# prototypefund/your-voice-TTS

Hardware: AMD Instinct MI355X
Metric: mel-frames/sec + RTF, Tacotron2 + 60-iter Griffin-Lim, LJSpeech (higher is better)
Workload: dtype f32; 1 GPU; configs[1]: Tacotron2 single sentence, HIP decoder loop + HIP Griffin-Lim 60 iters; sentences_per_gpu=1, L=100, gl_iters=60, model_config=config_tacotron2.json + forward_attn_mask (synthesize.py:86), parallelism=single GPU

## Files before the change

### your-voice-tts_amd/csrc/griffin_lim.hip

```cpp
#include <cmath>
#include <cstdio>
#include <cstdlib>
#include <string>
#include <type_traits>
#include <vector>

#include "gl_fft.h"

#ifndef GLP_SLEEP
#define GLP_SLEEP 1
#endif

using namespace tts;

namespace {

__device__ __forceinline__ double fval(float x) { return (double)x; }
__device__ __forceinline__ double fval(gran_t x) { return (double)__uint_as_float((unsigned)x.v); }
__device__ __forceinline__ void fstore(float* p, double v, unsigned) { *p = (float)v; }
__device__ __forceinline__ void fstore(gran_t* p, double v, unsigned tag) {
    p->v = ((unsigned long long)tag << 32) | (unsigned long long)__float_as_uint((float)v);
}

constexpr int MAG_KT = 64;
// ... 219 lines not shown
    for (int i = ilo; i <= ihi; ++i) {
        const int o = q - i * g.hop;
        y = (float)((double)y + fval(fr[(int64_t)i * g.winp + (o - g.fb)]));
        wss = (float)((double)wss + win2[o]);
    }
    return wss > 1.17549435e-38f ? y / wss : y;
}

constexpr int OLA_MAX = 5;
template <typename FT>
__device__ __forceinline__ float ola_sample_unrolled(const FT* __restrict__ fr, int q, int F, const Geo& g,
                                                     const double* __restrict__ win2) {
    if (q < g.woff) return 0.f;
    int ilo = q - g.woff - g.win + 1;
    ilo = ilo <= 0 ? 0 : (ilo + g.hop - 1) / g.hop;
    int ihi = (q - g.woff) / g.hop;
    if (ihi > F - 1) ihi = F - 1;
    double fv[OLA_MAX], wv[OLA_MAX];
#pragma unroll
    for (int k = 0; k < OLA_MAX; ++k) {
        const int i = ilo + k;
        const int o = q - i * g.hop;
        const bool ok = i <= ihi;
        fv[k] = ok ? fval(fr[(int64_t)i * g.winp + (o - g.fb)]) : 0.0;
        wv[k] = ok ? win2[o] : 0.0;
    }
    float y = 0.f, wss = 0.f;
#pragma unroll
    for (int k = 0; k < OLA_MAX; ++k) {
        y = (float)((double)y + fv[k]);
        wss = (float)((double)wss + wv[k]);
    }
    return wss > 1.17549435e-38f ? y / wss : y;
}

struct MagArgs {
    int mode;
    const float* spec;
    int n_in, Fmax;
    const int* F;
    const double* pinv;
    spec_t* S;
    float min_db, ref_db, power, max_norm;
    int signal_norm, symmetric, clip;
};

__device__ __forceinline__ float denorm_db(float x, const MagArgs& a) {
    float d = x;
    if (a.signal_norm) {
        if (a.symmetric) {
            if (a.clip) d = fminf(fmaxf(d, -a.max_norm), a.max_norm);
            d = ((d + a.max_norm) * -a.min_db / (2.f * a.max_norm)) + a.min_db;
        } else {
            if (a.clip) d = fminf(fmaxf(d, 0.f), a.max_norm);
            d = (d * -a.min_db / a.max_norm) + a.min_db;
        }
    }
    return (d + a.ref_db) * 0.05f;
}
__device__ __forceinline__ float denorm_to_amp(float x, const MagArgs& a) { return powf(10.f, denorm_db(x, a)); }
__device__ __forceinline__ float amp_of_db(float x, const MagArgs& a) { return exp10f(denorm_db(x, a)); }

constexpr int LIN_PER = 16;
__global__ __launch_bounds__(256) void gl_linear_magnitude_kernel(const MagArgs a) {
    const int b = blockIdx.y;
    const int64_t n = (int64_t)a.F[b] * NB;
// ... 598 lines not shown
        }
        if (lane == 0) {
            const int f = base + rank;
            sh[0] = f;
            sh[1] = f - 4 >= base && f + 4 < base + cnt && f >= 5 && f <= Fb - 6;
            if (!__all(ok)) fail(2);
        }
    }
    __syncthreads();
    if (sh[2]) return;
    const int f = sh[0];
    const bool local = sh[1];
    constexpr int PN = NFFT / GL_THREADS;
    const spec_t* Sf = a.S + ((int64_t)b * a.Fmax + f) * NB;
    std::conditional_t<TWO, TwMix, TwRegs> twf;
    twf.load(a.c.tw);
    __shared__ __align__(16) double2 tw_pass[TWO ? TW_LDS : 1];
    if constexpr (TWO) TwMix::fill(tw_pass, a.c.tw);
    double2 tk[4];
    spec_t sk[4];
#pragma unroll
    for (int r = 0; r < 4; ++r) {
        tk[r] = a.c.tw[bin2l(r)];
        sk[r] = Sf[bin2l(r)];
    }
    auto tkf = [&](int r) { return tk[r]; };
    const double2 tnyq = !TWO && tid == 0 ? a.c.tw[NH] : double2{0.0, 0.0};
    const spec_t snyq = tid == 0 ? Sf[NH] : 0.f;
    const int N = g.hop * (Fb - 1);
    extern __shared__ __align__(16) float og[];
    const int og_zero = GL_SLOTS * g.winp;
    __shared__ int rlo[GL_SLOTS], rhi[GL_SLOTS], rpre[GL_SLOTS + 1];
    if (tid < GL_SLOTS) {
        rlo[tid] = 0x7FFFFFFF;
        rhi[tid] = -1;
    }
    if (tid < 2) og[og_zero + tid] = 0.f;
    __syncthreads();
    double wi[PN];
    constexpr int OP = (OLA_MAX + 1) / 2;
    unsigned offp[PN][OP];
    float wssv[PN];
    if (og_zero > 0xFFFF) fail(6);
#pragma unroll
    for (int i = 0; i < PN; ++i) {
        const int n = edge_sample(tid, i);
        const bool sup = n >= g.woff && n < g.woff + g.win;
        wi[i] = sup ? a.c.win[n] : 0.0;
        const int q = reflect_idx(f * g.hop + n - NFFT / 2, N) + NFFT / 2;
        int ilo = q - g.woff - g.win + 1;
        ilo = ilo <= 0 ? 0 : (ilo + g.hop - 1) / g.hop;
        int ihi = (q - g.woff) / g.hop;
        if (ihi > Fb - 1) ihi = Fb - 1;
        const bool any = sup && q >= g.woff;
        float wss = 0.f;
#pragma unroll
        for (int k = 0; k < OP; ++k) offp[i][k] = 0u;
#pragma unroll
        for (int k = 0; k < OLA_MAX; ++k) {
            const int fi = ilo + k;
            const int o = q - fi * g.hop;
            const bool ok = any && fi <= ihi;
            const int sl = fi - f + GL_DMAX, gg = o - g.fb;
            if (ok && (sl < 0 || sl >= GL_SLOTS)) fail(4);
            const bool in = ok && sl >= 0 && sl < GL_SLOTS;
            offp[i][k >> 1] |= (unsigned)(in ? sl * g.winp + gg : og_zero) << (16 * (k & 1));
            if (in) {
                atomicMin(&rlo[sl], gg);
                atomicMax(&rhi[sl], gg);
            }
            wss = (float)((double)wss + (ok ? a.c.win2[o] : 0.0));
        }
        wssv[i] = wss > 1.17549435e-38f ? wss : 1.0f;
    }
    __syncthreads();
    if (tid == 0) {
        int acc = 0;
        for (int sl = 0; sl < GL_SLOTS; ++sl) {
            rpre[sl] = acc;
            acc += rhi[sl] >= 0 ? (rhi[sl] - (rlo[sl] & ~1)) / 2 + 1 : 0;
        }
        rpre[GL_SLOTS] = acc;
        if (acc > GL_PAIRS * GL_THREADS) fail(5);
    }
    __syncthreads();
    unsigned gdst[GL_PAIRS];
#pragma unroll
    for (int m = 0; m < GL_PAIRS; ++m) {
        const int u = tid + m * GL_THREADS;
        gdst[m] = (unsigned)og_zero;
        if (u < rpre[GL_SLOTS]) {
            int sl = 0;
            while (u >= rpre[sl + 1]) ++sl;
            const int g0 = (rlo[sl] & ~1) + 2 * (u - rpre[sl]);
            gdst[m] = (unsigned)(sl * g.winp + g0) | (g0 >= rlo[sl] ? 1u << 30 : 0u) | (g0 + 1 <= rhi[sl] ? 1u << 31 : 0u);
        }
    }
    const int gbase = (f - GL_DMAX) * g.winp * 8;
    auto goff = [&](int m) {
        return (gdst[m] >> 30) ? gbase + (int)(gdst[m] & 0x3FFFFFFFu) * 8 : GL_OOB_OFF;
    };
    auto soff_of = [&](int t, int i) {
        const int e = edge_sample(t, i);
// ... 74 lines not shown
        GL_PHASE(3)
        fft2l_inv(v, buf1, twf);
        GL_PHASE(4)
        if (b == 0 && f == p.drop_f) return;
        const unsigned nt = tag0 | (unsigned)(it + 1);
        const auto rD = buf_rsrc(dst, (unsigned)g.winp * 8);
#pragma unroll
        for (int r = 0; r < PN / 2; ++r) {
            const u32x4 gv = u32x4{__float_as_uint((float)(wi[2 * r] * (v[r].x * (1.0 / NH)))), nt,
                                   __float_as_uint((float)(wi[2 * r + 1] * (v[r].y * (1.0 / NH)))), nt};
            const int e = edge_sample(TWO ? tid_opaque() : tid, 2 * r);
            const int off = e + 1 >= g.woff && e < g.woff + g.win ? (e - g.fb) * 8 : GL_OOB_OFF;
            if (local) __builtin_amdgcn_raw_buffer_store_b128(gv, rD, off, 0, 0);
            else __builtin_amdgcn_raw_buffer_store_b128(gv, rD, off, 0, 0x10);
        }
        GL_PHASE(5)
    }
#undef GL_PHASE
    if (timed)
        for (int k = 0; k < 6; ++k) p.prof[k] = ph[k];
}
__global__ __launch_bounds__(GL_THREADS) void gl_persistent_kernel(const PersArgs p) { gl_persistent_body<false>(p); }
__global__ __launch_bounds__(GL_THREADS) __attribute__((amdgpu_waves_per_eu(2, 2))) void gl_persistent2_kernel(
    const PersArgs p) {
    gl_persistent_body<true>(p);
}

__global__ void gl_gran_to_frames_kernel(const gran_t* in, float* out, int64_t n) {
    const int64_t i = (int64_t)blockIdx.x * blockDim.x + threadIdx.x;
    if (i < n) out[i] = __uint_as_float((unsigned)in[i].v);
}

template <typename FT>
__global__ void gl_ola_kernel(const FinArgs a) {
    const int b = blockIdx.y;
    const int Fb = a.F[b];
    const int N = a.g.hop * (Fb - 1);
    const int p = blockIdx.x * blockDim.x + threadIdx.x;
    if (a.host_status && p == 0 && b == 0) {
        __hip_atomic_store(a.host_status, *a.status, __ATOMIC_RELAXED, __HIP_MEMORY_SCOPE_SYSTEM);
        if (a.host_seq) release_word_system(a.host_seq, a.seq);
    }
    if (p >= N) return;
    const bool bad = a.status && *a.status != 0;
    const FT* fr = static_cast<const FT*>(a.frames) + (int64_t)b * a.Fmax * a.g.winp;
    const Geo& g = a.g;
    const int q = p + NFFT / 2;
    float yv;
    if ((g.win + g.hop - 1) / g.hop <= OLA_MAX && q >= g.woff) {
        const int u = q - g.woff;
        const int ihu = u / g.hop;
        int ilo = u - g.win + 1;
        const bool full = ilo >= 1 && ihu <= Fb - 1;
        ilo = ilo <= 0 ? 0 : (ilo + g.hop - 1) / g.hop;
        const int ihi = ihu > Fb - 1 ? Fb - 1 : ihu;
        double fv[OLA_MAX];
#pragma unroll
        for (int k = 0; k < OLA_MAX; ++k) {
            const int i = ilo + k;
            fv[k] = i <= ihi ? fval(fr[(int64_t)i * g.winp + (q - i * g.hop - g.fb)]) : 0.0;
        }
        float y = 0.f, wss = 0.f;
#pragma unroll
        for (int k = 0; k < OLA_MAX; ++k) y = (float)((double)y + fv[k]);
        if (full) {
            wss = a.wssp[u - ihu * g.hop];
        } else {
            for (int i = ilo; i <= ihi; ++i) wss = (float)((double)wss + a.c.win2[q - i * g.hop]);
        }
        yv = wss > 1.17549435e-38f ? y / wss : y;
    } else {
        yv = ola_sample(fr, q, Fb, g, a.c.win2);
    }
    a.y[(int64_t)b * a.Nmax + p] = bad ? __builtin_nanf("") : yv;
}

constexpr int OLA_R = 4;
__device__ __forceinline__ int div_small(int n, int d, float rd) {
    int qt = (int)((float)n * rd);
    const int r = n - qt * d;
    qt += r >= d ? 1 : 0;
    qt -= r < 0 ? 1 : 0;
    return qt;
}
__global__ __launch_bounds__(256) void gl_ola_multi_kernel(const FinArgs a) {
    const int b = blockIdx.y;
    const int Fb = a.F[b];
    const Geo& g = a.g;
    const int N = g.hop * (Fb - 1);
    const int p0 = blockIdx.x * (256 * OLA_R) + threadIdx.x;
    if (a.host_status && p0 == 0 && b == 0) {
        __hip_atomic_store(a.host_status, *a.status, __ATOMIC_RELAXED, __HIP_MEMORY_SCOPE_SYSTEM);
        if (a.host_seq) release_word_system(a.host_seq, a.seq);
    }
    if (p0 >= N) return;
    const bool bad = a.status && *a.status != 0;
    const float* fr = static_cast<const float*>(a.frames) + (int64_t)b * a.Fmax * g.winp;
    const float rhop = __builtin_amdgcn_rcpf((float)g.hop);
    const int step = g.winp - g.hop;
    float fv[OLA_R][OLA_MAX], wv[OLA_R];
    int ilo[OLA_R], ihi[OLA_R];
#pragma unroll
    for (int j = 0; j < OLA_R; ++j) {
        const int q = p0 + 256 * j + NFFT / 2, u = q - g.woff;
        const int ihu = div_small(u, g.hop, rhop);
        int lo = u - g.win + 1;
        const bool full = lo >= 1 && ihu <= Fb - 1;
        lo = lo <= 0 ? 0 : div_small(lo + g.hop - 1, g.hop, rhop);
        const int hi = p0 + 256 * j < N ? min(ihu, Fb - 1) : -1;
        ilo[j] = lo;
        ihi[j] = hi;
        const int o = lo * step + q - g.fb;
#pragma unroll
        for (int k = 0; k < OLA_MAX; ++k) fv[j][k] = lo + k <= hi ? fr[o + k * step] : 0.f;
        wv[j] = full && hi >= 0 ? a.wssp[u - ihu * g.hop] : -1.f;
    }
#pragma unroll
// ... 29 lines not shown
__device__ __forceinline__ void scan_combine(double& A, double& Bv, double pa, double pb) {
    Bv = fma(pb, A, Bv);
    A = pa * A;
}
__global__ __launch_bounds__(SCAN_THREADS) void preemph_scan_kernel(const float* y, int64_t Nmax, const int* F, int hop,
                                                                    double coef, int apply, int64_t chunk, int64_t look,
                                                                    double* wav) {
    const int b = blockIdx.y;
    const int64_t N = (int64_t)hop * (F[b] - 1);
    const int64_t o0 = (int64_t)blockIdx.x * chunk;
    if (o0 >= N) return;
    const int64_t o1 = o0 + chunk < N ? o0 + chunk : N;
    const float* x = y + (int64_t)b * Nmax;
    double* o = wav + (int64_t)b * Nmax;
    const int tid = threadIdx.x, lane = tid & 63, wave = tid >> 6;
    if (!apply) {
        for (int64_t i = o0 + tid; i < o1; i += SCAN_THREADS) o[i] = (double)x[i];
        return;
    }
    constexpr int TILE = SCAN_THREADS * SCAN_PER, NW = SCAN_THREADS / 64;
    __shared__ double wa[NW], wb[NW];
    double cpow[SCAN_PER + 1];
    cpow[0] = 1.0;
#pragma unroll
    for (int k = 1; k <= SCAN_PER; ++k) cpow[k] = cpow[k - 1] * coef;
    const int64_t s0 = o0 - look > 0 ? ((o0 - look) & ~(int64_t)7) : 0;
    double carry = 0.0;
    for (int64_t t0 = s0; t0 < o1; t0 += TILE) {
        const int64_t base = t0 + (int64_t)tid * SCAN_PER;
        double v = 0.0, loc[SCAN_PER];
#pragma unroll
        for (int k = 0; k < SCAN_PER; ++k) {
            v = (base + k < o1 ? (double)x[base + k] : 0.0) + coef * v;
            loc[k] = v;
        }
        double A = cpow[SCAN_PER], Bv = v;
#pragma unroll
        for (int off = 1; off < 64; off <<= 1) {
            const double pa = __shfl_up(A, off, 64), pb = __shfl_up(Bv, off, 64);
            if (lane >= off) scan_combine(A, Bv, pa, pb);
        }
        if (lane == 63) { wa[wave] = A; wb[wave] = Bv; }
        __syncthreads();
        double WA = lane < NW ? wa[lane] : 1.0, WB = lane < NW ? wb[lane] : 0.0;
#pragma unroll
        for (int off = 1; off < NW; off <<= 1) {
            const double qa = __shfl_up(WA, off, 64), qb = __shfl_up(WB, off, 64);
            if (lane >= off) scan_combine(WA, WB, qa, qb);
        }
        const double win_in = wave == 0 ? carry : __shfl(WA, wave - 1, 64) * carry + __shfl(WB, wave - 1, 64);
        const double tile_end = __shfl(WA, NW - 1, 64) * carry + __shfl(WB, NW - 1, 64);
        const double pa = __shfl_up(A, 1, 64), pb = __shfl_up(Bv, 1, 64);
        const double cin = lane == 0 ? win_in : pa * win_in + pb;
#pragma unroll
        for (int k = 0; k < SCAN_PER; ++k) {
            const int64_t i = base + k;
            if (i >= o0 && i < o1) o[i] = loc[k] + cpow[k + 1] * cin;
        }
        carry = tile_end;
        __syncthreads();
    }
}

void launch_iteration(bool fused, bool wave, const IterArgs& a, hipStream_t s) {
    const dim3 grid(a.Fmax, a.B), block(GL_THREADS);
    if (fused) hipLaunchKernelGGL((gl_iter_kernel<false, true, frame_t>), grid, block, 0, s, a);
// ... 311 lines not shown
            } else {
                FinArgs o = c.fa;
                o.frames = frame_slot(g, c, i);
                launch_ola_frames(o, s);
            }
            launch_iteration(c.fused, g->wave, a, s);
        }
        hipError_t ce = hipGetLastError();
        hipError_t ee = hipStreamEndCapture(s, &graph);
        TTS_HIP(ce);
        TTS_HIP(ee);
        hipGraphExec_t exec = nullptr;
        TTS_HIP(hipGraphInstantiate(&exec, graph, nullptr, nullptr, 0));
        TTS_HIP(hipGraphDestroy(graph));
        it = g->graphs.emplace(key, exec).first;
    }
    TTS_HIP(hipGraphLaunch(it->second, s));
    return TTS_OK;
}

tts_status finish(tts_gl* g, RunCtx& c) {
    hipStream_t s = c.s;
    FinArgs& fa = c.fa;
    if (c.timed) TTS_HIP(hipEventRecord(g->ev_t1, s));
    fa.frames = c.persistent_ran ? static_cast<void*>(g->pgr.p + (size_t)(c.iters & 1) * c.fstride)
                                 : frame_slot(g, c, c.iters);
    fa.status = c.persistent_ran ? g->pstatus : nullptr;
    fa.host_status = c.persistent_ran ? g->host_status : nullptr;
    if (c.persistent_ran && !c.timed) {
        fa.host_seq = g->host_status + 1;
        fa.seq = ++g->seq;
        g->seq_stream = s;
    }
    if (c.persistent_ran)
        hipLaunchKernelGGL(gl_ola_kernel<gran_t>, dim3((c.Nmax + 255) / 256, c.B), dim3(256), 0, s, fa);
    else launch_ola_frames(fa, s);
    fa.status = nullptr;
    fa.host_status = nullptr;
    fa.host_seq = nullptr;
    TTS_HIP(hipGetLastError());
    const double cf = g->cfg.preemphasis, ac = std::fabs(cf);
    int64_t chunk = SCAN_CHUNK, look = 0;
    if (ac > 0.0) {
        const double need = ac < 1.0 ? std::ceil(std::log(1e-22) / std::log(ac)) : 1e30;
        if (need <= (double)(SCAN_THREADS * SCAN_PER - SCAN_CHUNK - 8)) look = (int64_t)need;
        else chunk = c.Nmax;
    }
    const dim3 sgrid((unsigned)((c.Nmax + chunk - 1) / chunk), c.B);
    hipLaunchKernelGGL(preemph_scan_kernel, sgrid, dim3(SCAN_THREADS), 0, s, g->y.p, c.Nmax, c.Fd, g->g.hop, cf,
                       cf != 0.0 ? 1 : 0, chunk, look, c.wav);
    TTS_HIP(hipGetLastError());
    return TTS_OK;
}

tts_status record_last(tts_gl* g, const RunCtx& c) {
    g->last_persistent = c.persistent_ran;
    g->last_path = c.persistent_ran ? TTS_GL_PATH_PERSISTENT : c.fused ? TTS_GL_PATH_FUSED : TTS_GL_PATH_UNFUSED;
    g->last_launches = c.persistent_ran ? 1 : (c.fused ? 1 : 2) * c.iters;
    if (c.timed) {
        TTS_HIP(hipEventRecord(g->ev_done, c.s));
        if (c.s != c.cs) TTS_HIP(hipStreamWaitEvent(c.cs, g->ev_done, 0));
    } else {
        g->last_ms = 0.f;
    }
    g->last_timed = c.timed;
    g->pending = true;
    if (!g->pipeline) TTS_TRY(gl_collect(g));
    g->last_fused = c.fused;
    g->have_last = true;
    g->last_iter = c.ia;
    g->last_fin = c.fa;
    g->last_fstride = c.fstride;
    return TTS_OK;
}

}

namespace tts {

bool gl_persistent_path(tts_gl* g, int B, int Fmax, int frames_total, int iters) {
    if (!(gl_fused_path(g, B, Fmax) && iters > 0 && iters < (1 << 14) && frames_total <= 512 && g->tmo > 0 &&
          !env_is("TTS_RESIDENT", '0')))
        return false;
// ... 106 lines not shown
```

### your-voice-tts_amd/csrc/resident_decoder.hip

```cpp
#include "handoff.h"
#include "resident.h"

namespace tts {
namespace {
using namespace handoff;

__device__ __forceinline__ float lstm_cell16(float pre, float& c) {
    const int k = threadIdx.x;
    const float act = (k >> 2) == 2 ? tanh_cell(pre) : sigmoid_cell(pre);
    const float f = dpp_move<0x104, 0xf>(act, 0.f);
    const float g = dpp_move<0x108, 0xf>(act, 0.f);
    const float o = dpp_move<0x10C, 0xf>(act, 0.f);
    const float c2 = f * c + act * g;
    c = c2;
    return o * tanh_cell(c2);
}
__device__ __forceinline__ float sigmoid_fast(float x) {
    return __builtin_amdgcn_rcpf(1.f + __builtin_amdgcn_exp2f(-x * 1.4426950408889634f));
}

__device__ __forceinline__ float dot4(float4 w, float4 x, float acc) {
    acc = fmaf(w.x, x.x, acc);
    acc = fmaf(w.y, x.y, acc);
    acc = fmaf(w.z, x.z, acc);
    return fmaf(w.w, x.w, acc);
}
__device__ __forceinline__ float4 ld4(const float* p) { return *reinterpret_cast<const float4*>(p); }
__device__ __forceinline__ void pin4(float4& a, float4& b, float4& c, float4& d) {
    asm volatile("" : "+v"(a.x), "+v"(a.y), "+v"(a.z), "+v"(a.w), "+v"(b.x), "+v"(b.y), "+v"(b.z), "+v"(b.w), "+v"(c.x),
                 "+v"(c.y), "+v"(c.z), "+v"(c.w), "+v"(d.x), "+v"(d.y), "+v"(d.z), "+v"(d.w));
}
__device__ __forceinline__ float sum32_dpp(float v) {
    v += dpp_move<0x111, 0xf>(v, 0.f);
    v += dpp_move<0x112, 0xf>(v, 0.f);
    v += dpp_move<0x114, 0xf>(v, 0.f);
    v += dpp_move<0x118, 0xf>(v, 0.f);
    v += dpp_move<0x142, 0xa>(v, 0.f);
    return v;
}

__device__ __forceinline__ int res_window(int k, int nn, int L) {
    if (k == 0) return nn >= 2 ? nn - 2 : nn - 2 + L;
    const int clo = nn >= 1 ? nn - 1 : L - 1, chi = min(nn + 2, L - 1);
    const int p = clo + k - 1;
    return p <= chi ? p : -1;
}
__device__ __forceinline__ int res_candidate(int s, int nn, int np, int L) {
    if (s < 5) return res_window(s, nn, L);
    if (s >= 15) return -1;
    const int p = res_window((s - 5) >> 1, np, L);
    if (p < 0) return -1;
    const int q = p + ((s - 5) & 1);
    return q < L ? q : -1;
}

__device__ __forceinline__ int res_part_slot(int sl, int k) { return sl * 32 + k; }

struct ResWin {
    int cx, clo, chi;
    bool in[4];
    bool iscx[4];
    bool pre, post;
};
// ... 340 lines not shown
            aa[i & 1] = dot4(wa[i], ld4(xh_att + (i - 6) * 128 + ks * 4), aa[i & 1]);                               \
        asm volatile("" ::: "memory");                         \
        _Pragma("unroll") for (int i = 10; i < 14; ++i)                                                             \
            aa[i & 1] = dot4(wa[i], ld4(xh_att + (i - 6) * 128 + ks * 4), aa[i & 1]);                               \
        out = aa[0] + aa[1];                                                                                        \
    }
#define RES_DEC_PARTIAL(out)                                                                                        \
    {                                                                                                               \
        float ad[2] = {0.f, 0.f};                                                                                   \
        _Pragma("unroll 2") for (int i = 8; i < 16; ++i)                                                            \
            ad[i & 1] = dot4(wdl[(i * 16 + r) * 32 + ks], ld4(xh_dec + (i - 8) * 128 + ks * 4), ad[i & 1]);         \
        out = ad[0] + ad[1];                                                                                        \
    }
    float acc_a_next = 0.f;
    if constexpr (!GEN) RES_ATT_PARTIAL(acc_a_next)
    int t = 0;
    for (;; ++t) {
        u64* G = a.gran + (t & 1) * GR_TOTAL;
        u64* const gxs = GEN ? Gx + (t & 1) * GR_TOTAL : G + s_x;
        u64* const gqs = GEN ? Gq + (t & 1) * GR_TOTAL : G + s_q;
        u64* const gcs = GEN ? Gc + (t & 1) * GR_TOTAL : G + s_c;
        u64* const g1s = GEN ? G1 + (t & 1) * GR_TOTAL : G + s_1;
        const unsigned E = (a.salt << 14) | (((unsigned)t & 2047u) << 3);
        const unsigned EP6 = ((a.salt << 14) | (((unsigned)(t - 1) & 2047u) << 3)) + 6u;
        float acc_a, acc_d;
        if constexpr (GEN) {
            RES_ATT_PARTIAL(acc_a)
            RES_DEC_PARTIAL(acc_d)
        } else {
            acc_a = acc_a_next;
        }
        if (tid == 0) { RES_EV(t, 12) }
        if (tid == 192) { RES_EV(t, 13) }
        if (wave < 3) {
            const int gp = s_1 + ((t & 1) ^ 1) * GR_TOTAL;
            bool ok = true;
            if (t == 0) {
                if (wave == 0) {
                    const float4 v = ld4(a.pre1 + lane * 4);
                    xp1[lane * 4] = v.x; xp1[lane * 4 + 1] = v.y; xp1[lane * 4 + 2] = v.z; xp1[lane * 4 + 3] = v.w;
                }
            } else {
                float p0 = 0.f, p1 = 0.f;
                for (int i = 0; i < a.sleep_p1; ++i) __builtin_amdgcn_s_sleep(4);
                if (wave < 2) {
                    ok = sweep_pair(rg, gp + 2 * pk, true, EP6, p0, p1, tmo);
                    xp1[2 * pk] = p0;
                    xp1[2 * pk + 1] = p1;
                } else {
                    ok = sweep_pair(rg, lane == 0 ? gp + PRE : -1, false, EP6, p0, p1, tmo);
                    if (lane == 0 && ok && p0 == 0.f) flags[0] = 1;
                }
            }
            RES_MARK(0);
            if (lane == 0 && !ok) { flags[1] = 1; fail(a.status, 1, t); }
        }
        __syncthreads();
        if (tid == 0) { RES_EV(t, 0) }
        if (flags[0] | flags[1]) break;
        {
            const float4 x = ld4(xp1 + lane * 4);
            u64* gx = gxs;
            if (has_row) {
                const float s0 = wave_sum_dpp(dot4(wp0, x, 0.f));
                if (lane == 0) publish_xcd(gx + r0, E + 1, fmaxf(s0 + bp2, 0.f));
            }
            RES_MARK(1);
            if (wave < 2) {
                for (int i = 0; i < a.sleep_pre2; ++i) __builtin_amdgcn_s_sleep(4);
                float q0, q1;
                const bool ok = sweep_pair(rg, s_x + (t & 1) * GR_TOTAL + 2 * pk, true, E + 1, q0, q1, tmo);
                xpre[2 * pk] = q0;
                xpre[2 * pk + 1] = q1;
                if (!ok && lane == 0) { flags[1] = 1; fail(a.status, 7, t); }
            }
        }
        __syncthreads();
        if (tid == 0) { RES_EV(t, 1) }
        if (flags[1]) break;
        RES_MARK(2);
#pragma unroll
        for (int i = 0; i < 2; ++i) acc_a = dot4(wa[i], ld4(xpre + i * 128 + ks * 4), acc_a);
        acc_a = sum32_dpp(acc_a);
        if (ks == 31) gates[r] = acc_a;
        if constexpr (!GEN) {
            if (t > 0) {
                if (wave >= RES_POLL_WAVES && wave < 2 * RES_POLL_WAVES) xrow[tid - 64 * RES_POLL_WAVES] = op_row;
                if (wave == 2 * RES_POLL_WAVES) xpt[lane] = op_pt;
            }
        }
        __syncthreads();
        RES_MARK(3);
        if (tid < 16) {
            float cs = st[32 + (tid & 3)];
            const float h = lstm_cell16(gates[tid] + st[tid], cs);
            if (tid < 4) {
                st[32 + tid] = cs;
                st[40 + tid] = h;
                publish(G + GR_HATT + 4 * c + tid, E + 2, h);
                if (tid == 0) { RES_EV(t, 2) }
            }
        }
        if constexpr (!GEN) {
            if (t > 0) {
                if (n == n_prev + 1 && n_prev >= 1) {
                    ex = erow[0];
                    erow[0] = erow[1];
                    erow[1] = erow[2];
                    erow[2] = erow[3];
                    if (wave < RES_POLL_WAVES) erow[3] = xrow[tid];
                    else erow[3] = op_own;
                } else if (n != n_prev) {
// ... 393 lines not shown
            if constexpr (!GEN) {
                RES_ATT_PARTIAL(acc_a_next)
                asm volatile("" : "+v"(acc_a_next));
            }
            for (int i = 0; i < a.sleep_hdec; ++i) __builtin_amdgcn_s_sleep(4);
            float h0, h1;
            const bool ok = sweep_pair(rg, (t & 1) * GR_TOTAL + GR_HDEC + 2 * pk, true, E + 5, h0, h1, tmo);
            xh_dec[2 * pk] = h0;
            xh_dec[2 * pk + 1] = h1;
            if (!ok && lane == 0) { flags[1] = 1; fail(a.status, 5, t); }
        }
        __syncthreads();
        if (tid == 0) { RES_EV(t, 6) }
        if (flags[1]) break;
        if constexpr (!GEN) {
            n_prev = n;
            n = flags[6];
        }
        if constexpr (GEN) {
            if (gf & GEN_TA) {
                float sta = gts[0];
#pragma unroll
                for (int k = 1; k < RES_WAVES; ++k) sta += gts[k];
                gu = sigmoidf_(sta + gtb);
            }
        }
        RES_MARK(12);
        long long m0 = 0;
        if (prof && tid == 128) m0 = (long long)wall_clock64();
        {
            const bool stw = stop_cu && wave == 3;
            const float4* wsr = reinterpret_cast<const float4*>(rm) + 6 * 64 + lane;
            float s = 0.f, ss = 0.f;
#pragma unroll
            for (int i = 0; i < 4; ++i) {
                const float4 x = ld4(xh_dec + i * 256 + lane * 4);
                s = dot4(w1[i], x, s);
                if (stw) ss = dot4(wsr[i * 64], x, ss);
            }
#pragma unroll
            for (int i = 4; i < 6; ++i) {
                const float4 x = ld4(xctx + (i - 4) * 256 + lane * 4);
                s = dot4(w1[i], x, s);
                if (stw) ss = dot4(wsr[i * 64], x, ss);
            }
            s = wave_sum_dpp(s);
            u64* g1 = g1s;
            if (has_row && lane == 0) {
                const float p = fmaxf(s + bp1, 0.f);
                publish_xcd(g1 + r0, E + 6, p);
                if (wave == 0) { RES_EV(t, 7) }
                if (xlog) a.pre1[r0] = p;
            }
            if (stw) {
                ss = wave_sum_dpp(ss);
                if (lane == 0) {
                    const float stv = sigmoidf_(ss + st[49]);
                    if (xlog && t < a.hist_cap) a.stop_hist[t] = stv;
                    const float tail = xctx[ENC];
                    int* sst = reinterpret_cast<int*>(st);
                    const int f1 = sst[50] | ((tail > 0.8f && t > L) ? 1 : 0);
                    sst[50] = f1;
                    int nd = 0;
                    if (f1 && t > 2 * L) {
                        sst[51] += 1;
                        if (sst[51] > 20) nd = 1;
                    } else if (t + 1 == a.max_steps) {
                        nd = 1;
                    }
                    if (!nd && t + 1 >= a.hist_cap) {
                        nd = 1;
                        fail(a.status, 100);
                    }
                    if (nd && xlog) {
                        a.done[0] = 1;
                        a.n_steps[0] = t + 1;
                    }
                    publish_xcd(g1 + PRE, E + 6, nd ? 0.f : 1.f);
                }
            }
        }
        if (prof && tid == 128) pacc[13] += (long long)wall_clock64() - m0;
        if constexpr (!GEN) {
            if (wave >= RES_POLL_WAVES) {
                if (n == n_prev + 1 && n_prev >= 1) {
                    const int ro = n + 2 <= L - 1 ? ((n + 2) * ENC + tid) * 4 : OOB_OFF;
                    op_own = __uint_as_float(__builtin_amdgcn_raw_buffer_load_b32(renc, ro, 0, VOLATILE_AUX));
                    if (wave < 2 * RES_POLL_WAVES)
                        op_row = __uint_as_float(__builtin_amdgcn_raw_buffer_load_b32(
                            renc, n + 2 <= L - 1 ? ro - 256 * RES_POLL_WAVES : OOB_OFF, 0, VOLATILE_AUX));
                }
                if (wave == 2 * RES_POLL_WAVES) {
                    const int pos = res_candidate(lane & 15, n, n_prev, L);
                    op_pt = __uint_as_float(__builtin_amdgcn_raw_buffer_load_b32(
                        rpt, pos >= 0 ? ((rank + 32 * (lane >> 4)) * a.Lcap + pos) * 4 : OOB_OFF, 0, VOLATILE_AUX));
                    if (lane == 0) { RES_EV(t, 14) }
                }
            }
        }
    }
    if (flags[1]) return;
    if (wave == 4 && t > 0) mel_row(t - 1);
    if (prof && tid == 0)
        for (int k = 0; k < RES_PHASES; ++k) a.prof[(c == 0 ? 0 : 1) * RES_PHASES + k] = pacc[k];
    const int pl = (t - 1) & 1;
    if (tid < 4) {
        a.h_att[pl * a.hps + 4 * c + tid] = st[40 + tid];
        a.c_att[4 * c + tid] = st[32 + tid];
        a.h_dec[pl * a.hps + 4 * c + tid] = st[44 + tid];
        a.c_dec[4 * c + tid] = st[36 + tid];
    }
// ... 118 lines not shown
```

Before: 109,100 mel-frames/s.

## Fuse final overlap-add and de-emphasis scan into one epilogue kernel

For single-sentence batches, a new epilogue kernel replaces the separate final overlap-add kernel and the preemphasis scan kernel. It computes OLA samples tile by tile into shared memory and scans them directly, removing one launch and the global round trip of the intermediate signal. Separately, the persistent kernel's per-slot frame range setup now uses a closed-form reflection bound instead of shared-memory atomics, and it swaps integer divisions by hop for reciprocal-based division. The fused path redoes OLA over the look-back overlap region and adds more code paths that must stay consistent.

```diff
diff --git a/your-voice-tts_amd/csrc/griffin_lim.hip b/your-voice-tts_amd/csrc/griffin_lim.hip
--- a/your-voice-tts_amd/csrc/griffin_lim.hip
+++ b/your-voice-tts_amd/csrc/griffin_lim.hip
@@ -275,6 +275,14 @@
         wss = (float)((double)wss + wv[k]);
     }
     return wss > 1.17549435e-38f ? y / wss : y;
+}
+
+__device__ __forceinline__ int div_small(int n, int d, float rd) {
+    int qt = (int)((float)n * rd);
+    const int r = n - qt * d;
+    qt += r >= d ? 1 : 0;
+    qt -= r < 0 ? 1 : 0;
+    return qt;
 }
 
 struct MagArgs {
@@ -939,8 +947,27 @@
     const int og_zero = GL_SLOTS * g.winp;
     __shared__ int rlo[GL_SLOTS], rhi[GL_SLOTS], rpre[GL_SLOTS + 1];
     if (tid < GL_SLOTS) {
-        rlo[tid] = 0x7FFFFFFF;
-        rhi[tid] = -1;
+        int lo = 0x7FFFFFFF, hi = -1;
+        const int fi = f + tid - GL_DMAX;
+        if (fi >= 0 && fi < Fb) {
+            const int pa = f * g.hop + g.woff - NFFT / 2, pb = pa + g.win - 1;
+            int rmin = 0, rmax = 0;
+            if (N > 1) {
+                const int period = 2 * (N - 1);
+                auto ahead = [&](int x) { const int m = x % period; return m > 0 ? period - m : -m; };
+                const int ra = reflect_idx(pa, N), rb = reflect_idx(pb, N);
+                rmin = pa + ahead(pa) <= pb ? 0 : min(ra, rb);
+                rmax = pa + ahead(pa - (N - 1)) <= pb ? N - 1 : max(ra, rb);
+            }
+            const int q0 = max(rmin + NFFT / 2, fi * g.hop + g.woff);
+            const int q1 = min(rmax + NFFT / 2, fi * g.hop + g.woff + g.win - 1);
+            if (q0 <= q1) {
+                lo = q0 - fi * g.hop - g.fb;
+                hi = q1 - fi * g.hop - g.fb;
+            }
+        }
+        rlo[tid] = lo;
+        rhi[tid] = hi;
     }
     if (tid < 2) og[og_zero + tid] = 0.f;
     __syncthreads();
@@ -949,6 +976,7 @@
     unsigned offp[PN][OP];
     float wssv[PN];
     if (og_zero > 0xFFFF) fail(6);
+    const float rhop = __builtin_amdgcn_rcpf((float)g.hop);
 #pragma unroll
     for (int i = 0; i < PN; ++i) {
         const int n = edge_sample(tid, i);
@@ -956,8 +984,8 @@
         wi[i] = sup ? a.c.win[n] : 0.0;
         const int q = reflect_idx(f * g.hop + n - NFFT / 2, N) + NFFT / 2;
         int ilo = q - g.woff - g.win + 1;
-        ilo = ilo <= 0 ? 0 : (ilo + g.hop - 1) / g.hop;
-        int ihi = (q - g.woff) / g.hop;
+        ilo = ilo <= 0 ? 0 : div_small(ilo + g.hop - 1, g.hop, rhop);
+        int ihi = div_small(q - g.woff, g.hop, rhop);
         if (ihi > Fb - 1) ihi = Fb - 1;
         const bool any = sup && q >= g.woff;
         float wss = 0.f;
@@ -972,10 +1000,6 @@
             if (ok && (sl < 0 || sl >= GL_SLOTS)) fail(4);
             const bool in = ok && sl >= 0 && sl < GL_SLOTS;
             offp[i][k >> 1] |= (unsigned)(in ? sl * g.winp + gg : og_zero) << (16 * (k & 1));
-            if (in) {
-                atomicMin(&rlo[sl], gg);
-                atomicMax(&rhi[sl], gg);
-            }
             wss = (float)((double)wss + (ok ? a.c.win2[o] : 0.0));
         }
         wssv[i] = wss > 1.17549435e-38f ? wss : 1.0f;
@@ -1116,6 +1140,35 @@
 }
 
 template <typename FT>
+__device__ __forceinline__ float ola_final_sample(const FinArgs& a, const FT* __restrict__ fr, int Fb, int p) {
+    const Geo& g = a.g;
+    const int q = p + NFFT / 2;
+    if ((g.win + g.hop - 1) / g.hop <= OLA_MAX && q >= g.woff) {
+        const int u = q - g.woff;
+        const int ihu = u / g.hop;
+        int ilo = u - g.win + 1;
+        const bool full = ilo >= 1 && ihu <= Fb - 1;
+        ilo = ilo <= 0 ? 0 : (ilo + g.hop - 1) / g.hop;
+        const int ihi = ihu > Fb - 1 ? Fb - 1 : ihu;
+        double fv[OLA_MAX];
+#pragma unroll
+        for (int k = 0; k < OLA_MAX; ++k) {
+            const int i = ilo + k;
+            fv[k] = i <= ihi ? fval(fr[(int64_t)i * g.winp + (q - i * g.hop - g.fb)]) : 0.0;
+        }
+        float y = 0.f, wss = 0.f;
+#pragma unroll
+        for (int k = 0; k < OLA_MAX; ++k) y = (float)((double)y + fv[k]);
+        if (full) {
+            wss = a.wssp[u - ihu * g.hop];
+        } else {
+            for (int i = ilo; i <= ihi; ++i) wss = (float)((double)wss + a.c.win2[q - i * g.hop]);
+        }
+        return wss > 1.17549435e-38f ? y / wss : y;
+    }
+    return ola_sample(fr, q, Fb, g, a.c.win2);
+}
+template <typename FT>
 __global__ void gl_ola_kernel(const FinArgs a) {
     const int b = blockIdx.y;
     const int Fb = a.F[b];
@@ -1128,45 +1181,11 @@
     if (p >= N) return;
     const bool bad = a.status && *a.status != 0;
     const FT* fr = static_cast<const FT*>(a.frames) + (int64_t)b * a.Fmax * a.g.winp;
-    const Geo& g = a.g;
-    const int q = p + NFFT / 2;
-    float yv;
-    if ((g.win + g.hop - 1) / g.hop <= OLA_MAX && q >= g.woff) {
-        const int u = q - g.woff;
-        const int ihu = u / g.hop;
-        int ilo = u - g.win + 1;
-        const bool full = ilo >= 1 && ihu <= Fb - 1;
-        ilo = ilo <= 0 ? 0 : (ilo + g.hop - 1) / g.hop;
-        const int ihi = ihu > Fb - 1 ? Fb - 1 : ihu;
-        double fv[OLA_MAX];
-#pragma unroll
-        for (int k = 0; k < OLA_MAX; ++k) {
-            const int i = ilo + k;
-            fv[k] = i <= ihi ? fval(fr[(int64_t)i * g.winp + (q - i * g.hop - g.fb)]) : 0.0;
-        }
-        float y = 0.f, wss = 0.f;
-#pragma unroll
-        for (int k = 0; k < OLA_MAX; ++k) y = (float)((double)y + fv[k]);
-        if (full) {
-            wss = a.wssp[u - ihu * g.hop];
-        } else {
-            for (int i = ilo; i <= ihi; ++i) wss = (float)((double)wss + a.c.win2[q - i * g.hop]);
-        }
-        yv = wss > 1.17549435e-38f ? y / wss : y;
-    } else {
-        yv = ola_sample(fr, q, Fb, g, a.c.win2);
-    }
+    const float yv = ola_final_sample(a, fr, Fb, p);
     a.y[(int64_t)b * a.Nmax + p] = bad ? __builtin_nanf("") : yv;
 }
 
 constexpr int OLA_R = 4;
-__device__ __forceinline__ int div_small(int n, int d, float rd) {
-    int qt = (int)((float)n * rd);
-    const int r = n - qt * d;
-    qt += r >= d ? 1 : 0;
-    qt -= r < 0 ? 1 : 0;
-    return qt;
-}
 __global__ __launch_bounds__(256) void gl_ola_multi_kernel(const FinArgs a) {
     const int b = blockIdx.y;
     const int Fb = a.F[b];
@@ -1262,6 +1281,116 @@
 #pragma unroll
         for (int k = 0; k < SCAN_PER; ++k) {
             v = (base + k < o1 ? (double)x[base + k] : 0.0) + coef * v;
+            loc[k] = v;
+        }
+        double A = cpow[SCAN_PER], Bv = v;
+#pragma unroll
+        for (int off = 1; off < 64; off <<= 1) {
+            const double pa = __shfl_up(A, off, 64), pb = __shfl_up(Bv, off, 64);
+            if (lane >= off) scan_combine(A, Bv, pa, pb);
+        }
+        if (lane == 63) { wa[wave] = A; wb[wave] = Bv; }
+        __syncthreads();
+        double WA = lane < NW ? wa[lane] : 1.0, WB = lane < NW ? wb[lane] : 0.0;
+#pragma unroll
+        for (int off = 1; off < NW; off <<= 1) {
+            const double qa = __shfl_up(WA, off, 64), qb = __shfl_up(WB, off, 64);
+            if (lane >= off) scan_combine(WA, WB, qa, qb);
+        }
+        const double win_in = wave == 0 ? carry : __shfl(WA, wave - 1, 64) * carry + __shfl(WB, wave - 1, 64);
+        const double tile_end = __shfl(WA, NW - 1, 64) * carry + __shfl(WB, NW - 1, 64);
+        const double pa = __shfl_up(A, 1, 64), pb = __shfl_up(Bv, 1, 64);
+        const double cin = lane == 0 ? win_in : pa * win_in + pb;
+#pragma unroll
+        for (int k = 0; k < SCAN_PER; ++k) {
+            const int64_t i = base + k;
+            if (i >= o0 && i < o1) o[i] = loc[k] + cpow[k + 1] * cin;
+        }
+        carry = tile_end;
+        __syncthreads();
+    }
+}
+
+__device__ __forceinline__ float fraw(float x) { return x; }
+__device__ __forceinline__ float fraw(gran_t x) { return __uint_as_float((unsigned)x.v); }
+template <typename FT>
+__device__ __forceinline__ void ola_final_tile(const FinArgs& a, const FT* __restrict__ fr, int Fb, int p0, int lim,
+                                               bool bad, float* xs) {
+    const Geo& g = a.g;
+    const float rhop = __builtin_amdgcn_rcpf((float)g.hop);
+    const int step = g.winp - g.hop;
+    float fv[SCAN_PER][OLA_MAX], wv[SCAN_PER];
+    int ilo[SCAN_PER], ihi[SCAN_PER];
+#pragma unroll
+    for (int j = 0; j < SCAN_PER; ++j) {
+        const int q = p0 + SCAN_THREADS * j + NFFT / 2, u = q - g.woff;
+        const int ihu = div_small(u, g.hop, rhop);
+        int lo = u - g.win + 1;
+        const bool full = lo >= 1 && ihu <= Fb - 1;
+        lo = lo <= 0 ? 0 : div_small(lo + g.hop - 1, g.hop, rhop);
+        const int hi = p0 + SCAN_THREADS * j < lim ? min(ihu, Fb - 1) : -1;
+        ilo[j] = lo;
+        ihi[j] = hi;
+        const int o = lo * step + q - g.fb;
+#pragma unroll
+        for (int k = 0; k < OLA_MAX; ++k) fv[j][k] = lo + k <= hi ? fraw(fr[o + k * step]) : 0.f;
+        wv[j] = full && hi >= 0 ? a.wssp[u - ihu * g.hop] : -1.f;
+    }
+#pragma unroll
+    for (int j = 0; j < SCAN_PER; ++j) {
+        const int q = p0 + SCAN_THREADS * j + NFFT / 2;
+        float y = 0.f;
+#pragma unroll
+        for (int k = 0; k < OLA_MAX; ++k) y = (float)((double)y + (double)fv[j][k]);
+        float wss = wv[j];
+        if (wss < 0.f) {
+            wss = 0.f;
+            for (int i = ilo[j]; i <= ihi[j]; ++i) wss = (float)((double)wss + a.c.win2[q - i * g.hop]);
+        }
+        const float yv = wss > 1.17549435e-38f ? y / wss : y;
+        xs[SCAN_THREADS * j] = ihi[j] < 0 ? 0.f : bad ? __builtin_nanf("") : yv;
+    }
+}
+
+template <typename FT>
+__global__ __launch_bounds__(SCAN_THREADS) void gl_epilogue_kernel(const FinArgs a, double coef, int apply, int64_t chunk,
+                                                                   int64_t look, double* wav) {
+    const int b = blockIdx.y;
+    const int Fb = a.F[b];
+    const int64_t N = (int64_t)a.g.hop * (Fb - 1);
+    const int64_t o0 = (int64_t)blockIdx.x * chunk;
+    const int tid = threadIdx.x, lane = tid & 63, wave = tid >> 6;
+    if (a.host_status && blockIdx.x == 0 && b == 0 && tid == 0) {
+        __hip_atomic_store(a.host_status, *a.status, __ATOMIC_RELAXED, __HIP_MEMORY_SCOPE_SYSTEM);
+        if (a.host_seq) release_word_system(a.host_seq, a.seq);
+    }
+    if (o0 >= N) return;
+    const int64_t o1 = o0 + chunk < N ? o0 + chunk : N;
+    const bool bad = a.status && *a.status != 0;
+    const FT* fr = static_cast<const FT*>(a.frames) + (int64_t)b * a.Fmax * a.g.winp;
+    auto sample = [&](int64_t i) { return bad ? __builtin_nanf("") : ola_final_sample(a, fr, Fb, (int)i); };
+    double* o = wav + (int64_t)b * a.Nmax;
+    if (!apply) {
+        for (int64_t i = o0 + tid; i < o1; i += SCAN_THREADS) o[i] = (double)sample(i);
+        return;
+    }
+    constexpr int TILE = SCAN_THREADS * SCAN_PER, NW = SCAN_THREADS / 64;
+    __shared__ float xs[TILE];
+    __shared__ double wa[NW], wb[NW];
+    double cpow[SCAN_PER + 1];
+    cpow[0] = 1.0;
+#pragma unroll
+    for (int k = 1; k <= SCAN_PER; ++k) cpow[k] = cpow[k - 1] * coef;
+    const int64_t s0 = o0 - look > 0 ? ((o0 - look) & ~(int64_t)7) : 0;
+    double carry = 0.0;
+    for (int64_t t0 = s0; t0 < o1; t0 += TILE) {
+        ola_final_tile(a, fr, Fb, (int)t0 + tid, (int)o1, bad, xs + tid);
+        __syncthreads();
+        const int64_t base = t0 + (int64_t)tid * SCAN_PER;
+        double v = 0.0, loc[SCAN_PER];
+#pragma unroll
+        for (int k = 0; k < SCAN_PER; ++k) {
+            v = (double)xs[tid * SCAN_PER + k] + coef * v;
             loc[k] = v;
         }
         double A = cpow[SCAN_PER], Bv = v;
@@ -1639,23 +1768,30 @@
         fa.seq = ++g->seq;
         g->seq_stream = s;
     }
-    if (c.persistent_ran)
+    const double cf = g->cfg.preemphasis, ac = std::fabs(cf);
+    int64_t chunk = SCAN_CHUNK, look = 0;
+    if (ac > 0.0) {
+        const double need = ac < 1.0 ? std::ceil(std::log(1e-22) / std::log(ac)) : 1e30;
+        if (need <= (double)(SCAN_THREADS * SCAN_PER - SCAN_CHUNK - 8)) look = (int64_t)need;
+        else chunk = c.Nmax;
+    }
+    const dim3 sgrid((unsigned)((c.Nmax + chunk - 1) / chunk), c.B);
+    const int apply = cf != 0.0 ? 1 : 0;
+    const bool one = c.B == 1 && (c.persistent_ran || c.fused) && !env_is("TTS_GL_EPILOGUE", '0');
+    if (one && c.persistent_ran)
+        hipLaunchKernelGGL(gl_epilogue_kernel<gran_t>, sgrid, dim3(SCAN_THREADS), 0, s, fa, cf, apply, chunk, look, c.wav);
+    else if (one)
+        hipLaunchKernelGGL(gl_epilogue_kernel<frame_t>, sgrid, dim3(SCAN_THREADS), 0, s, fa, cf, apply, chunk, look, c.wav);
+    else if (c.persistent_ran)
         hipLaunchKernelGGL(gl_ola_kernel<gran_t>, dim3((c.Nmax + 255) / 256, c.B), dim3(256), 0, s, fa);
     else launch_ola_frames(fa, s);
     fa.status = nullptr;
     fa.host_status = nullptr;
     fa.host_seq = nullptr;
     TTS_HIP(hipGetLastError());
-    const double cf = g->cfg.preemphasis, ac = std::fabs(cf);
-    int64_t chunk = SCAN_CHUNK, look = 0;
-    if (ac > 0.0) {
-        const double need = ac < 1.0 ? std::ceil(std::log(1e-22) / std::log(ac)) : 1e30;
-        if (need <= (double)(SCAN_THREADS * SCAN_PER - SCAN_CHUNK - 8)) look = (int64_t)need;
-        else chunk = c.Nmax;
-    }
-    const dim3 sgrid((unsigned)((c.Nmax + chunk - 1) / chunk), c.B);
-    hipLaunchKernelGGL(preemph_scan_kernel, sgrid, dim3(SCAN_THREADS), 0, s, g->y.p, c.Nmax, c.Fd, g->g.hop, cf,
-                       cf != 0.0 ? 1 : 0, chunk, look, c.wav);
+    if (one) return TTS_OK;
+    hipLaunchKernelGGL(preemph_scan_kernel, sgrid, dim3(SCAN_THREADS), 0, s, g->y.p, c.Nmax, c.Fd, g->g.hop, cf, apply,
+                       chunk, look, c.wav);
     TTS_HIP(hipGetLastError());
     return TTS_OK;
 }
```

Result: no change. 109,700 mel-frames/s, median of 6 (+0.5%).

## Defer stop-flag poll off critical path and split stop-token dot product

Applied to the files above, without the earlier changes.

In the non-GEN resident decoder, the stop/done flag poll moves out of the first barrier phase into wave 2 during the prenet-2 phase. The loop exit check is delayed by one barrier, so the prenet-1 sweep no longer waits on the stop CU's publish. The layer-1 dot product is restructured into register-pinned batches of three loads. The stop-token dot product now runs only after the main pre1 value is published, shortening the stop CU's critical path. Extra profiling events are added, and the deferred exit adds a small amount of speculative work on the final step.

```diff
diff --git a/your-voice-tts_amd/csrc/resident_decoder.hip b/your-voice-tts_amd/csrc/resident_decoder.hip
--- a/your-voice-tts_amd/csrc/resident_decoder.hip
+++ b/your-voice-tts_amd/csrc/resident_decoder.hip
@@ -29,6 +29,10 @@
 __device__ __forceinline__ void pin4(float4& a, float4& b, float4& c, float4& d) {
     asm volatile("" : "+v"(a.x), "+v"(a.y), "+v"(a.z), "+v"(a.w), "+v"(b.x), "+v"(b.y), "+v"(b.z), "+v"(b.w), "+v"(c.x),
                  "+v"(c.y), "+v"(c.z), "+v"(c.w), "+v"(d.x), "+v"(d.y), "+v"(d.z), "+v"(d.w));
+}
+__device__ __forceinline__ void pin3(float4& a, float4& b, float4& c) {
+    asm volatile("" : "+v"(a.x), "+v"(a.y), "+v"(a.z), "+v"(a.w), "+v"(b.x), "+v"(b.y), "+v"(b.z), "+v"(b.w), "+v"(c.x),
+                 "+v"(c.y), "+v"(c.z), "+v"(c.w));
 }
 __device__ __forceinline__ float sum32_dpp(float v) {
     v += dpp_move<0x111, 0xf>(v, 0.f);
@@ -435,7 +439,8 @@
         }
         if (tid == 0) { RES_EV(t, 12) }
         if (tid == 192) { RES_EV(t, 13) }
-        if (wave < 3) {
+        constexpr bool DEFER = !GEN;
+        if (wave < (DEFER ? 2 : 3)) {
             const int gp = s_1 + ((t & 1) ^ 1) * GR_TOTAL;
             bool ok = true;
             if (t == 0) {
@@ -450,9 +455,15 @@
                     ok = sweep_pair(rg, gp + 2 * pk, true, EP6, p0, p1, tmo);
                     xp1[2 * pk] = p0;
                     xp1[2 * pk + 1] = p1;
+                    if constexpr (!GEN) {
+                        if (lane == 0 && wave == (rank & 1) && !stop_cu) { RES_EV(t, 11) }
+                    }
                 } else {
                     ok = sweep_pair(rg, lane == 0 ? gp + PRE : -1, false, EP6, p0, p1, tmo);
                     if (lane == 0 && ok && p0 == 0.f) flags[0] = 1;
+                    if constexpr (!GEN) {
+                        if (lane == 0) { RES_EV(t, 15) }
+                    }
                 }
             }
             RES_MARK(0);
@@ -460,7 +471,7 @@
         }
         __syncthreads();
         if (tid == 0) { RES_EV(t, 0) }
-        if (flags[0] | flags[1]) break;
+        if (DEFER ? flags[1] : (flags[0] | flags[1])) break;
         {
             const float4 x = ld4(xp1 + lane * 4);
             u64* gx = gxs;
@@ -469,6 +480,17 @@
                 if (lane == 0) publish_xcd(gx + r0, E + 1, fmaxf(s0 + bp2, 0.f));
             }
             RES_MARK(1);
+            if constexpr (DEFER) {
+                if (wave == 2 && t > 0) {
+                    float p0 = 0.f, p1 = 0.f;
+                    const bool ok = sweep_pair(rg, lane == 0 ? s_1 + ((t & 1) ^ 1) * GR_TOTAL + PRE : -1, false, EP6, p0, p1, tmo);
+                    if (lane == 0) {
+                        if (!ok) { flags[1] = 1; fail(a.status, 1, t); }
+                        else if (p0 == 0.f) flags[0] = 1;
+                        RES_EV(t, 15)
+                    }
+                }
+            }
             if (wave < 2) {
                 for (int i = 0; i < a.sleep_pre2; ++i) __builtin_amdgcn_s_sleep(4);
                 float q0, q1;
@@ -480,7 +502,7 @@
         }
         __syncthreads();
         if (tid == 0) { RES_EV(t, 1) }
-        if (flags[1]) break;
+        if (DEFER ? (flags[0] | flags[1]) : flags[1]) break;
         RES_MARK(2);
 #pragma unroll
         for (int i = 0; i < 2; ++i) acc_a = dot4(wa[i], ld4(xpre + i * 128 + ks * 4), acc_a);
@@ -940,17 +962,30 @@
             const bool stw = stop_cu && wave == 3;
             const float4* wsr = reinterpret_cast<const float4*>(rm) + 6 * 64 + lane;
             float s = 0.f, ss = 0.f;
-#pragma unroll
-            for (int i = 0; i < 4; ++i) {
-                const float4 x = ld4(xh_dec + i * 256 + lane * 4);
-                s = dot4(w1[i], x, s);
-                if (stw) ss = dot4(wsr[i * 64], x, ss);
-            }
-#pragma unroll
-            for (int i = 4; i < 6; ++i) {
-                const float4 x = ld4(xctx + (i - 4) * 256 + lane * 4);
-                s = dot4(w1[i], x, s);
-                if (stw) ss = dot4(wsr[i * 64], x, ss);
+            if constexpr (!GEN) {
+#pragma unroll
+                for (int h = 0; h < 6; h += 3) {
+                    float4 xx[3];
+#pragma unroll
+                    for (int j = 0; j < 3; ++j)
+                        xx[j] = h + j < 4 ? ld4(xh_dec + (h + j) * 256 + lane * 4) : ld4(xctx + (h + j - 4) * 256 + lane * 4);
+                    pin3(xx[0], xx[1], xx[2]);
+#pragma unroll
+                    for (int j = 0; j < 3; ++j) s = dot4(w1[h + j], xx[j], s);
+                }
+            } else {
+#pragma unroll
+                for (int i = 0; i < 4; ++i) {
+                    const float4 x = ld4(xh_dec + i * 256 + lane * 4);
+                    s = dot4(w1[i], x, s);
+                    if (stw) ss = dot4(wsr[i * 64], x, ss);
+                }
+#pragma unroll
+                for (int i = 4; i < 6; ++i) {
+                    const float4 x = ld4(xctx + (i - 4) * 256 + lane * 4);
+                    s = dot4(w1[i], x, s);
+                    if (stw) ss = dot4(wsr[i * 64], x, ss);
+                }
             }
             s = wave_sum_dpp(s);
             u64* g1 = g1s;
@@ -961,6 +996,23 @@
                 if (xlog) a.pre1[r0] = p;
             }
             if (stw) {
+                if constexpr (!GEN) {
+                    asm volatile("" ::: "memory");
+#pragma unroll 1
+                    for (int h = 0; h < 6; h += 3) {
+                        float4 wv[3], xx[3];
+#pragma unroll
+                        for (int j = 0; j < 3; ++j) {
+                            const int i = h + j;
+                            wv[j] = wsr[i * 64];
+                            xx[j] = i < 4 ? ld4(xh_dec + i * 256 + lane * 4) : ld4(xctx + (i - 4) * 256 + lane * 4);
+                        }
+                        pin3(wv[0], wv[1], wv[2]);
+                        pin3(xx[0], xx[1], xx[2]);
+#pragma unroll
+                        for (int j = 0; j < 3; ++j) ss = dot4(wv[j], xx[j], ss);
+                    }
+                }
                 ss = wave_sum_dpp(ss);
                 if (lane == 0) {
                     const float stv = sigmoidf_(ss + st[49]);
@@ -985,6 +1037,7 @@
                         a.n_steps[0] = t + 1;
                     }
                     publish_xcd(g1 + PRE, E + 6, nd ? 0.f : 1.f);
+                    if constexpr (!GEN) { RES_EV(t, 11) }
                 }
             }
         }
```

New measurement: 109,600 mel-frames/s before, 112,300 mel-frames/s after (median of 6 runs). +2.5%, better.
